# HansBambel/SmaAt-UNet

Measured on NVIDIA H100. Metric: SmaAt-UNet fwd frames/sec @ B=32 12×288×288; depthwise % HBM roofline, higher is better.
Workload: dtype f32

## Files before the change

### smaat_unet_b200/csrc/dsconv_fused.cu

```cuda
#include <stdlib.h>

#include "tc_common.cuh"

namespace smaat {

struct DsParams {
  const float* dw_w;
  const float* dw_b;
  const float* scale;
  const float* shift;
  float* y;
  int64_t y_bstride;
  double* stats;
  const float* oc_w;
  const float* oc_b;
  float* oc_y;
  int C0, C1, H, W, Cout, relu, K;
  int tiles_x, tiles_y, npass, total_tiles, nchunks;
};

template <int N_TILE, int KPL, int PW, bool X3>
struct DsCfg {
  static constexpr int PH = TC_BM / PW;
  static constexpr int BW = PW + 8, BH = PH + 2;
  static constexpr int CC = TC_BK / KPL;
  static constexpr int IN_BYTES = CC * BH * BW * 4;
  static constexpr int A_BYTES = TC_BM * TC_BK * 4;
  static constexpr int B_BYTES = N_TILE * TC_BK * 4;
  static constexpr int AST_BYTES = (X3 ? 2 : 1) * A_BYTES;
  static constexpr int BST_BYTES = (X3 ? 2 : 1) * B_BYTES;
  static constexpr int OFF_ALO = A_BYTES;
  static constexpr int OFF_BLO = B_BYTES;
  static constexpr int AS = X3 ? (N_TILE > 64 ? 2 : 3) : 4;
  static constexpr int NG = N_TILE > 64 ? 1 : 2;
  static constexpr int BS = X3 ? 2 : 4;
  static constexpr int AFF_N = 512;
  static constexpr int BAR_BYTES = 512;
  static constexpr int IS_FIT = (224 * 1024 - 1024 - BAR_BYTES - 3 * AFF_N * 4 - AS * AST_BYTES - BS * BST_BYTES) / IN_BYTES;
  static constexpr int IS = IS_FIT > 8 ? 8 : IS_FIT;
  static constexpr int OFF_A = ((IS * IN_BYTES + 1023) / 1024) * 1024;
  static constexpr int OFF_BR = OFF_A + AS * AST_BYTES;
  static constexpr int OFF_BAR = OFF_BR + BS * BST_BYTES;
  static_assert((IS * NG + IS + 2 * AS + 2 * BS) * 8 <= BAR_BYTES, "barrier block");
  static constexpr int TOTAL = OFF_BAR + BAR_BYTES + 3 * AFF_N * 4 + 1024;
  static constexpr uint32_t B_TX = BST_BYTES;
  static constexpr int PROD_WARP = 12;
  static constexpr int THREADS = 384 + 128 * NG;
  static_assert(IS >= 2, "input ring");
  static_assert(NG <= AS, "phase-parity barriers");
  static_assert(IN_BYTES % 128 == 0, "TMA destination alignment");
  static_assert(TOTAL <= 227 * 1024, "shared memory budget");
};

template <int N_TILE, int KPL, int PW, bool X3, bool A_SMEM>
__global__ void __launch_bounds__(DsCfg<N_TILE, KPL, PW, X3>::THREADS, 1)
    dsconv_fused_kernel(const __grid_constant__ CUtensorMap map_in0, const __grid_constant__ CUtensorMap map_in1,
                        const __grid_constant__ CUtensorMap map_w, const __grid_constant__ CUtensorMap map_wlo,
                        const DsParams p) {
  using L = DsCfg<N_TILE, KPL, PW, X3>;
  constexpr int PH = L::PH, BW = L::BW, BH = L::BH, CC = L::CC, IS = L::IS, AS = L::AS, BS = L::BS;
  extern __shared__ __align__(1024) unsigned char smem_dyn[];
  unsigned char* smem = smem_dyn + ((1024u - (smem_u32(smem_dyn) & 1023u)) & 1023u);
  unsigned char* a_base = smem + L::OFF_A;
  unsigned char* b_base = smem + L::OFF_BR;
  uint64_t* bars = reinterpret_cast<uint64_t*>(smem + L::OFF_BAR);
  uint64_t* in_full = bars;
  uint64_t* in_empty = in_full + IS * L::NG;
  uint64_t* a_full = in_empty + IS;
  uint64_t* a_empty = a_full + AS;
  uint64_t* b_full = a_empty + AS;
  uint64_t* b_empty = b_full + BS;
  float* aff = reinterpret_cast<float*>(smem + L::OFF_BAR + L::BAR_BYTES);

  const int warp = __shfl_sync(0xffffffffu, (int)(threadIdx.x >> 5), 0);
  const int lane = threadIdx.x & 31;
  const int nch = p.nchunks;
  const int tiles_per_img = p.tiles_x * p.tiles_y * p.npass;
  auto decode = [&](int tile, int& b, int& ty, int& tx, int& np) {
    b = tile / tiles_per_img;
    int t2 = tile - b * tiles_per_img;
    np = t2 % p.npass;
    t2 /= p.npass;
    ty = t2 / p.tiles_x;
    tx = t2 - ty * p.tiles_x;
  };

  if (warp == 0 && lane == 0) {
    tma_prefetch_desc(&map_in0);
    tma_prefetch_desc(&map_in1);
    tma_prefetch_desc(&map_w);
    if (X3) tma_prefetch_desc(&map_wlo);
    for (int s = 0; s < IS; ++s) {
      for (int g = 0; g < L::NG; ++g) mbar_init(&in_full[s * L::NG + g], 1);
      mbar_init(&in_empty[s], 128);
    }
    for (int s = 0; s < AS; ++s) {
      mbar_init(&a_full[s], 128);
      mbar_init(&a_empty[s], 8);
    }
    for (int s = 0; s < BS; ++s) {
      mbar_init(&b_full[s], 1);
      mbar_init(&b_empty[s], 8);
    }
    fence_barrier_init();
  }
  for (int c = threadIdx.x; c < L::AFF_N; c += blockDim.x) {
    aff[c] = (c < p.Cout && p.scale) ? __ldg(p.scale + c) : 1.f;
    aff[L::AFF_N + c] = (c < p.Cout && p.shift) ? __ldg(p.shift + c) : 0.f;
    aff[2 * L::AFF_N + c] = (c < p.Cout && p.oc_w) ? __ldg(p.oc_w + c) : 0.f;
  }
  __syncthreads();

  if (warp == 0) {
    if (lane == 0) {
      uint32_t gc = 0;
      for (int tile = blockIdx.x; tile < p.total_tiles; tile += gridDim.x) {
        int b, ty, tx, np;
        decode(tile, b, ty, tx, np);
        const int x0 = tx * PW, y0 = ty * PH;
        for (int i = 0; i < nch; ++i, ++gc) {
          const int s = gc % IS;
          mbar_wait(&in_empty[s], ((gc / IS) & 1u) ^ 1u);
          uint64_t* full = &in_full[s * L::NG + (int)(gc % (uint32_t)L::NG)];
          mbar_arrive_expect_tx(full, L::IN_BYTES);
          const int cb = i * CC;
          const CUtensorMap* m = (cb < p.C0) ? &map_in0 : &map_in1;
          const int cc = (cb < p.C0) ? cb : cb - p.C0;
          asm volatile(
              "cp.async.bulk.tensor.4d.shared::cluster.global.mbarrier::complete_tx::bytes [%0], [%1, {%3, %4, %5, %6}], [%2];" ::
                  "r"(smem_u32(smem + s * L::IN_BYTES)),
              "l"(reinterpret_cast<uint64_t>(m)), "r"(smem_u32(full)), "r"(x0 - 4), "r"(y0 - 1), "r"(cc), "r"(b)
              : "memory");
        }
      }
    }
    return;
  }
  if (warp == 1) {
    if (lane == 0) {
      uint32_t gc = 0;
      for (int tile = blockIdx.x; tile < p.total_tiles; tile += gridDim.x) {
        int b, ty, tx, np;
        decode(tile, b, ty, tx, np);
        for (int i = 0; i < nch; ++i, ++gc) {
          const int sb = gc % BS;
          mbar_wait(&b_empty[sb], ((gc / BS) & 1u) ^ 1u);
          mbar_arrive_expect_tx(&b_full[sb], L::B_TX);
          tma_load_2d(b_base + sb * L::BST_BYTES, &map_w, &b_full[sb], i * TC_BK, np * N_TILE);
          if (X3) tma_load_2d(b_base + sb * L::BST_BYTES + L::OFF_BLO, &map_wlo, &b_full[sb], i * TC_BK, np * N_TILE);
        }
      }
    }
    return;
  }
  if (warp < 4) return;

  if (warp < L::PROD_WARP) {
    const int wg = (warp >> 2) - 1, wq = warp & 3;
    const int g = lane >> 2, t = lane & 3;
    const int m0 = A_SMEM ? 64 * wg + 16 * wq + g : tc_row_pixel(wg, wq, 0, g);
    const int m1 = A_SMEM ? m0 + 8 : tc_row_pixel(wg, wq, 1, g);
    const float act_lo = p.relu ? 0.f : -INFINITY;
    const int64_t P = (int64_t)p.H * p.W;
    uint32_t gc = 0;
    for (int tile = blockIdx.x; tile < p.total_tiles; tile += gridDim.x) {
      int b, ty, tx, np;
      decode(tile, b, ty, tx, np);
      float acc[N_TILE / 2];
#pragma unroll
      for (int i = 0; i < N_TILE / 2; ++i) acc[i] = 0.f;
      for (int i = 0; i < nch; ++i, ++gc) {
        const int sa = gc % AS, sb = gc % BS;
        mbar_wait(&a_full[sa], (gc / AS) & 1u);
        mbar_wait(&b_full[sb], (gc / BS) & 1u);
        const unsigned char* ast = a_base + sa * L::AST_BYTES;
        const uint64_t bd0 = make_kmajor_desc(smem_u32(b_base + sb * L::BST_BYTES));
        const uint64_t bl0 = make_kmajor_desc(smem_u32(b_base + sb * L::BST_BYTES + L::OFF_BLO));
        if (A_SMEM) {
          const uint32_t a_addr = smem_u32(ast) + (uint32_t)(wg * 64 * 128);
          const uint64_t ad0 = make_kmajor_desc(a_addr), al0 = make_kmajor_desc(a_addr + L::OFF_ALO);
          wgmma_fence();
#pragma unroll
          for (int kk = 0; kk < TC_BK / 8; ++kk) {
            Wgmma<N_TILE>::ss(acc, ad0 + (uint64_t)(2 * kk), bd0 + (uint64_t)(2 * kk), 1u);
            if (X3) {
              Wgmma<N_TILE>::ss(acc, al0 + (uint64_t)(2 * kk), bd0 + (uint64_t)(2 * kk), 1u);
              Wgmma<N_TILE>::ss(acc, ad0 + (uint64_t)(2 * kk), bl0 + (uint64_t)(2 * kk), 1u);
            }
          }
        } else {
#pragma unroll
        for (int kk = 0; kk < TC_BK / 8; ++kk) {
          float vh[4], vl[4];
          load_a_frag(ast, kk, t, m0, m1, vh);
          if (X3) load_a_frag(ast + L::OFF_ALO, kk, t, m0, m1, vl);
          uint32_t ahi[4], alo[4];
#pragma unroll
          for (int e = 0; e < 4; ++e) {
            ahi[e] = __float_as_uint(vh[e]);
            alo[e] = X3 ? __float_as_uint(vl[e]) : 0u;
          }
          wgmma_fence();
          Wgmma<N_TILE>::rs(acc, ahi, bd0 + (uint64_t)(2 * kk), 1u);
          if (X3) {
            Wgmma<N_TILE>::rs(acc, alo, bd0 + (uint64_t)(2 * kk), 1u);
            Wgmma<N_TILE>::rs(acc, ahi, bl0 + (uint64_t)(2 * kk), 1u);
          }
        }
        }
        wgmma_commit();
        wgmma_wait0();
        wgmma_keep(acc);
        __syncwarp();
        if (lane == 0) {
          mbar_arrive(&a_empty[sa]);
          mbar_arrive(&b_empty[sb]);
        }
      }

      const int n0 = np * N_TILE;
      const int gy0 = ty * PH + m0 / PW, gx0 = tx * PW + m0 % PW;
      const int gy1 = ty * PH + m1 / PW, gx1 = tx * PW + m1 % PW;
      const bool v0 = gy0 < p.H && gx0 < p.W, v1 = gy1 < p.H && gx1 < p.W;
      const int64_t o0 = (int64_t)gy0 * p.W + gx0, o1 = (int64_t)gy1 * p.W + gx1;
      if (p.stats) {
        const double npix = (double)((__popc(__ballot_sync(0xffffffffu, v0)) + __popc(__ballot_sync(0xffffffffu, v1))) / 4);
#pragma unroll
        for (int j = 0; j < N_TILE / 8; ++j) {
#pragma unroll
          for (int e = 0; e < 2; ++e) {
            const float a = v0 ? acc[4 * j + e] : 0.f, bb = v1 ? acc[4 * j + 2 + e] : 0.f;
            const float s1 = frag_colsum(a + bb), s2 = frag_colsum(fmaf(a, a, bb * bb));
            const int c = 8 * j + 2 * t + e;
            if (lane < 4 && c < p.Cout) {
              const double sc = (double)aff[c], sh = (double)aff[L::AFF_N + c];
              atomicAdd(p.stats + c, sc * (double)s1 + npix * sh);
              atomicAdd(p.stats + p.Cout + c, sc * sc * (double)s2 + 2.0 * sc * sh * (double)s1 + npix * sh * sh);
            }
          }
        }
      }
      if (p.oc_y) {
        float d0 = 0.f, d1 = 0.f;
#pragma unroll
        for (int j = 0; j < N_TILE / 8; ++j) {
#pragma unroll
          for (int e = 0; e < 2; ++e) {
            const int c = 8 * j + 2 * t + e;
            const float sc = aff[c], sh = aff[L::AFF_N + c], w = aff[2 * L::AFF_N + c];
            d0 = fmaf(fmaxf(fmaf(acc[4 * j + e], sc, sh), act_lo), w, d0);
            d1 = fmaf(fmaxf(fmaf(acc[4 * j + 2 + e], sc, sh), act_lo), w, d1);
          }
        }
        d0 += __shfl_xor_sync(0xffffffffu, d0, 1);
        d0 += __shfl_xor_sync(0xffffffffu, d0, 2);
        d1 += __shfl_xor_sync(0xffffffffu, d1, 1);
        d1 += __shfl_xor_sync(0xffffffffu, d1, 2);
        const float ob = p.oc_b ? __ldg(p.oc_b) : 0.f;
        if (t == 0) {
          if (v0) p.oc_y[(int64_t)b * P + o0] = d0 + ob;
          if (v1) p.oc_y[(int64_t)b * P + o1] = d1 + ob;
        }
      } else {
        float* yb = p.y + (int64_t)b * p.y_bstride;
#pragma unroll
        for (int j = 0; j < N_TILE / 8; ++j) {
#pragma unroll
          for (int e = 0; e < 2; ++e) {
            const int c = n0 + 8 * j + 2 * t + e;
            if (c < p.Cout) {
              const float sc = aff[c], sh = aff[L::AFF_N + c];
              float* yc = yb + (int64_t)c * P;
              if (v0) yc[o0] = fmaxf(fmaf(acc[4 * j + e], sc, sh), act_lo);
              if (v1) yc[o1] = fmaxf(fmaf(acc[4 * j + 2 + e], sc, sh), act_lo);
            }
          }
        }
      }
    }
    return;
  }

  {
    const int g = (warp - L::PROD_WARP) >> 2;
    const int t = threadIdx.x - 32 * L::PROD_WARP - 128 * g;
    const int Cin = p.C0 + p.C1;
    uint32_t gc = 0, iph = 0;
    for (int tile = blockIdx.x; tile < p.total_tiles; tile += gridDim.x) {
      for (int i = 0; i < nch; ++i, ++gc) {
        if ((int)(gc % (uint32_t)L::NG) != g) continue;
        const int s = gc % IS;
        float wr[KPL][9], br[KPL];
        auto task_channel = [&](int task) { return (PW == 32) ? (task >> 3) : (((task >> 4) << 1) | ((task >> 2) & 1)); };
        auto load_weights = [&](int task) {
          const int gch = i * CC + task_channel(task);
          const bool chv = gch < Cin;
#pragma unroll
          for (int kk = 0; kk < KPL; ++kk) {
            const int gk = gch * KPL + kk;
#pragma unroll
            for (int w9 = 0; w9 < 9; ++w9) wr[kk][w9] = chv ? __ldg(p.dw_w + (int64_t)gk * 9 + w9) : 0.f;
            br[kk] = (chv && p.dw_b) ? __ldg(p.dw_b + gk) : 0.f;
          }
        };
        load_weights(t);
        mbar_wait(&in_full[s * L::NG + g], (iph >> s) & 1u);
        iph ^= 1u << s;
        const int sa = gc % AS;
        mbar_wait(&a_empty[sa], ((gc / AS) & 1u) ^ 1u);
        unsigned char* my_op = a_base + sa * L::AST_BYTES;
        const float* in_stage = reinterpret_cast<const float*>(smem + s * L::IN_BYTES);
#pragma unroll 1
        for (int task = t; task < CC * 8; task += 128) {
          int ci, qc, rg;
          if (PW == 32) {
            ci = task >> 3; qc = task & 7; rg = 0;
          } else {
            qc = task & 3; ci = ((task >> 4) << 1) | ((task >> 2) & 1); rg = (task >> 3) & 1;
          }
          constexpr int NQ = PW / 4;
          const int c0 = qc << 2, r0 = rg << 2;
          if (task != t) load_weights(task);
          const float* trow = in_stage + (ci * BH + r0) * BW + c0 + 3;
          float win[3][6];
          const bool lb = (qc == 0), rb = (qc == NQ - 1);
          const int edge = lb ? 0 : 5;
          auto load_row = [&](float* wl, int r) {
            const float4 a = *reinterpret_cast<const float4*>(trow + r * BW + 1);
            float left = __shfl_up_sync(0xffffffffu, a.w, 1), right = __shfl_down_sync(0xffffffffu, a.x, 1);
            if (lb | rb) {
              const float e = trow[r * BW + edge];
              if (lb) left = e; else right = e;
            }
            wl[0] = left; wl[1] = a.x; wl[2] = a.y; wl[3] = a.z; wl[4] = a.w; wl[5] = right;
          };
#pragma unroll
          for (int r = 0; r < 2; ++r) load_row(win[r], r);
#pragma unroll
          for (int rr = 0; rr < 4; ++rr) {
            load_row(win[(rr + 2) % 3], rr + 2);
            const float* w0 = win[rr % 3];
            const float* w1 = win[(rr + 1) % 3];
            const float* w2 = win[(rr + 2) % 3];
            const int m = (r0 + rr) * PW + c0;
#pragma unroll
            for (int kk = 0; kk < KPL; ++kk) {
              float o4[4];
#pragma unroll
              for (int j = 0; j < 4; ++j) {
                float a = br[kk];
                a = fmaf(wr[kk][0], w0[j], a); a = fmaf(wr[kk][1], w0[j + 1], a); a = fmaf(wr[kk][2], w0[j + 2], a);
                a = fmaf(wr[kk][3], w1[j], a); a = fmaf(wr[kk][4], w1[j + 1], a); a = fmaf(wr[kk][5], w1[j + 2], a);
                a = fmaf(wr[kk][6], w2[j], a); a = fmaf(wr[kk][7], w2[j + 1], a); a = fmaf(wr[kk][8], w2[j + 2], a);
                o4[j] = a;
              }
              if (A_SMEM) {
                const int kr = ci * KPL + kk;
#pragma unroll
                for (int j = 0; j < 4; ++j) {
                  const uint32_t off = kmajor_offset(m + j, kr);
                  const float h = X3 ? tf32_hi(o4[j]) : o4[j];
                  *reinterpret_cast<float*>(my_op + off) = h;
                  if (X3) *reinterpret_cast<float*>(my_op + L::OFF_ALO + off) = o4[j] - h;
                }
                continue;
              }
              const uint32_t off = a_tile_offset(ci * KPL + kk, m);
              if (X3) {
                const float4 h = make_float4(tf32_hi(o4[0]), tf32_hi(o4[1]), tf32_hi(o4[2]), tf32_hi(o4[3]));
                *reinterpret_cast<float4*>(my_op + off) = h;
                *reinterpret_cast<float4*>(my_op + L::OFF_ALO + off) = make_float4(o4[0] - h.x, o4[1] - h.y, o4[2] - h.z, o4[3] - h.w);
              } else {
                *reinterpret_cast<float4*>(my_op + off) = make_float4(o4[0], o4[1], o4[2], o4[3]);
              }
            }
          }
        }
        if (A_SMEM) fence_proxy_async_smem();
        mbar_arrive(&a_full[sa]);
        mbar_arrive(&in_empty[s]);
      }
    }
  }
}

template <int N_TILE, int KPL, int PW, bool X3, bool A_SMEM>
static int launch_ds(const CUtensorMap& m0, const CUtensorMap& m1, const CUtensorMap& mw, const CUtensorMap& mwl, DsParams p,
                     int B, cudaStream_t st) {
  using L = DsCfg<N_TILE, KPL, PW, X3>;
  auto kern = dsconv_fused_kernel<N_TILE, KPL, PW, X3, A_SMEM>;
  static std::atomic<uint64_t> attr_mask{0};
  if (first_use_on_device(attr_mask)) {
    cudaError_t e = cudaFuncSetAttribute(kern, cudaFuncAttributeMaxDynamicSharedMemorySize, L::TOTAL);
    if (e != cudaSuccess) return fail(SMAAT_E_CUDA, "dsconv: smem attribute (%d B): %s", L::TOTAL, cudaGetErrorString(e));
  }
  p.tiles_x = ceil_div(p.W, PW);
  p.tiles_y = ceil_div(p.H, L::PH);
  p.npass = ceil_div(p.Cout, N_TILE);
  const int64_t total = (int64_t)B * p.tiles_x * p.tiles_y * p.npass;
  SMAAT_REQUIRE(total < (1ll << 31), "dsconv: too many tiles");
  p.total_tiles = (int)total;
  p.nchunks = ceil_div(p.C0 + p.C1, L::CC);
  const int grid = p.total_tiles < num_sms() ? p.total_tiles : num_sms();
  kern<<<grid, L::THREADS, L::TOTAL, st>>>(m0, m1, mw, mwl, p);
  SMAAT_LAUNCH_CHECK("smaat_dsconv_fwd");
  return SMAAT_OK;
}

static int pick_pw(int H, int W) {
  double best = 1e9;
  int pw = 0;
  const int cand[2] = {32, 16};
  for (int i = 0; i < 2; ++i) {
    const int c = cand[i], ph = TC_BM / c;
    const double waste = ((double)ceil_div(W, c) * c / W) * ((double)ceil_div(H, ph) * ph / H);
    if (waste < best - 1e-9) {
      best = waste;
      pw = c;
    }
  }
  return best <= 1.35 ? pw : 0;
}

static bool ds_eligible(const float* x0, int C0, int64_t bs0, const float* x1, int C1, int64_t bs1, const float* pw_w,
                        const float* pw_w_lo, int H, int W, int k, int Cout, bool stats, bool outconv) {
  if (k != 1 && k != 2) return false;
  if (Cout < 8 || Cout > 512 || (Cout > 128 && (Cout % 128 != 0 || stats || outconv))) return false;
  if (W % 4 != 0 || !aligned16(x0) || bs0 % 4 != 0) return false;
  if (C1 > 0 && (!aligned16(x1) || bs1 % 4 != 0 || C0 % (TC_BK / k) != 0)) return false;
  const int K = k * (C0 + C1);
  if (K % 4 != 0 || !aligned16(pw_w) || (pw_w_lo && !aligned16(pw_w_lo))) return false;
  return pick_pw(H, W) != 0;
}

static std::atomic<int> g_ds_impl{-1};
static int ds_impl() {
  int v = g_ds_impl.load(std::memory_order_relaxed);
  if (v < 0) {
    const char* e = getenv("SMAAT_DS_IMPL");
    v = e ? atoi(e) : 0;
    if (v < 0 || v > 2) v = 0;
    g_ds_impl.store(v, std::memory_order_relaxed);
  }
  return v;
}

}

using namespace smaat;

extern "C" int smaat_set_dsconv_impl(int impl) {
  SMAAT_REQUIRE(impl >= 0 && impl <= 2, "set_dsconv_impl: 0 = auto, 1 = A operand from shared memory, 2 = A operand from registers");
  g_ds_impl.store(impl, std::memory_order_relaxed);
  return SMAAT_OK;
}

extern "C" int smaat_dsconv_eligible2(const float* x0, int C0, int64_t x0_bstride, const float* x1, int C1, int64_t x1_bstride,
                                      const float* pw_w, int H, int W, int k, int Cout, int with_stats) {
  return ds_eligible(x0, C0, x0_bstride, x1, C1, x1_bstride, pw_w, nullptr, H, W, k, Cout, with_stats != 0, false) ? 1 : 0;
}

extern "C" int smaat_dsconv_eligible(const float* x0, int C0, int64_t x0_bstride, const float* x1, int C1, int64_t x1_bstride,
                                     const float* pw_w, int H, int W, int k, int Cout) {
  return smaat_dsconv_eligible2(x0, C0, x0_bstride, x1, C1, x1_bstride, pw_w, H, W, k, Cout, 0);
}

static int dsconv_run(const float* x0, int C0, int64_t x0_bstride, const float* x1, int C1, int64_t x1_bstride, const float* dw_w,
                      const float* dw_b, const float* pw_w, const float* pw_w_lo, const float* scale, const float* shift, float* y,
                      int64_t y_bstride, double* stats, const float* oc_w, const float* oc_b, float* oc_y, int B, int H, int W,
                      int k, int Cout, int relu, int mode, void* stream) {
  SMAAT_REQUIRE(x0 && dw_w && pw_w && (y || oc_y), "dsconv: null pointer");
  SMAAT_REQUIRE(B > 0 && C0 > 0 && C1 >= 0 && H > 0 && W > 0 && Cout > 0, "dsconv: bad shape");
  SMAAT_REQUIRE(C1 == 0 || x1, "dsconv: C1=%d but x1 is null", C1);
  SMAAT_REQUIRE(mode == SMAAT_PW_TF32 || mode == SMAAT_PW_TF32X3, "dsconv: mode must be SMAAT_PW_TF32 or SMAAT_PW_TF32X3");
  SMAAT_REQUIRE(mode != SMAAT_PW_TF32X3 || pw_w_lo, "dsconv: TF32X3 needs pw_w_lo (see smaat_split_tf32)");
  SMAAT_REQUIRE(oc_y || y_bstride >= (int64_t)Cout * H * W, "dsconv: y batch stride too small");
  SMAAT_REQUIRE(!oc_y || (oc_w && !stats), "dsconv+outconv: needs the OutConv weight and no batch statistics");
  if (!ds_eligible(x0, C0, x0_bstride, x1, C1, x1_bstride, pw_w, pw_w_lo, H, W, k, Cout, stats != nullptr, oc_y != nullptr))
    return fail(SMAAT_E_UNSUPPORTED, "dsconv: shape not taken by the fused kernel (k=%d Cout=%d H=%d W=%d); use dw3x3 + pw1x1", k,
                Cout, H, W);
  cudaStream_t st = (cudaStream_t)stream;
  const int pw = pick_pw(H, W);
  const int ph = TC_BM / pw;
  const int n_tile = Cout > 64 ? 128 : 64;
  const int cc = TC_BK / k;
  const bool x3 = mode == SMAAT_PW_TF32X3;
  const bool a_smem = ds_impl() == 1;
  const int K = k * (C0 + C1);

  CUtensorMap m0, m1, mw, mwl;
  const uint32_t box[4] = {(uint32_t)(pw + 8), (uint32_t)(ph + 2), (uint32_t)cc, 1u};
  {
    const uint64_t dims[4] = {(uint64_t)W, (uint64_t)H, (uint64_t)C0, (uint64_t)B};
    const uint64_t str[4] = {0, (uint64_t)W * 4, (uint64_t)H * W * 4, (uint64_t)x0_bstride * 4};
    int r = make_tmap_f32(&m0, x0, 4, dims, str, box, CU_TENSOR_MAP_SWIZZLE_NONE, "dsconv(x0)");
    if (r) return r;
    m1 = m0;
  }
  if (C1 > 0) {
    const uint64_t dims[4] = {(uint64_t)W, (uint64_t)H, (uint64_t)C1, (uint64_t)B};
    const uint64_t str[4] = {0, (uint64_t)W * 4, (uint64_t)H * W * 4, (uint64_t)x1_bstride * 4};
    int r = make_tmap_f32(&m1, x1, 4, dims, str, box, CU_TENSOR_MAP_SWIZZLE_NONE, "dsconv(x1)");
    if (r) return r;
  }
  {
    const uint64_t dims[2] = {(uint64_t)K, (uint64_t)Cout};
    const uint64_t str[2] = {0, (uint64_t)K * 4};
    const uint32_t wbox[2] = {(uint32_t)TC_BK, (uint32_t)n_tile};
    int r = make_tmap_f32(&mw, pw_w, 2, dims, str, wbox, CU_TENSOR_MAP_SWIZZLE_128B, "dsconv(w)");
    if (r) return r;
    mwl = mw;
    if (x3) {
      r = make_tmap_f32(&mwl, pw_w_lo, 2, dims, str, wbox, CU_TENSOR_MAP_SWIZZLE_128B, "dsconv(w_lo)");
      if (r) return r;
    }
  }
  DsParams p;
  p.dw_w = dw_w; p.dw_b = dw_b; p.scale = scale; p.shift = shift; p.y = y; p.y_bstride = y_bstride; p.stats = stats;
  p.oc_w = oc_w; p.oc_b = oc_b; p.oc_y = oc_y;
  p.C0 = C0; p.C1 = C1; p.H = H; p.W = W; p.Cout = Cout; p.relu = relu; p.K = K;
  p.tiles_x = p.tiles_y = p.npass = p.total_tiles = p.nchunks = 0;

#define DS_DISPATCH(NT, KP, PWv)                                                                           \
  return x3 ? (a_smem ? launch_ds<NT, KP, PWv, true, true>(m0, m1, mw, mwl, p, B, st)                       \
                      : launch_ds<NT, KP, PWv, true, false>(m0, m1, mw, mwl, p, B, st))                     \
            : (a_smem ? launch_ds<NT, KP, PWv, false, true>(m0, m1, mw, mwl, p, B, st)                      \
                      : launch_ds<NT, KP, PWv, false, false>(m0, m1, mw, mwl, p, B, st))
  if (n_tile == 64) {
    if (k == 2) { if (pw == 32) { DS_DISPATCH(64, 2, 32); } else { DS_DISPATCH(64, 2, 16); } }
    else        { if (pw == 32) { DS_DISPATCH(64, 1, 32); } else { DS_DISPATCH(64, 1, 16); } }
  } else {
    if (k == 2) { if (pw == 32) { DS_DISPATCH(128, 2, 32); } else { DS_DISPATCH(128, 2, 16); } }
    else        { if (pw == 32) { DS_DISPATCH(128, 1, 32); } else { DS_DISPATCH(128, 1, 16); } }
  }
#undef DS_DISPATCH
}

extern "C" int smaat_dsconv_fwd(const float* x0, int C0, int64_t x0_bstride, const float* x1, int C1, int64_t x1_bstride,
                                const float* dw_w, const float* dw_b, const float* pw_w, const float* pw_w_lo,
                                const float* scale, const float* shift, float* y, int64_t y_bstride, double* stats, int B, int H,
                                int W, int k, int Cout, int relu, int mode, void* stream) {
  SMAAT_REQUIRE(y, "dsconv: null output");
  return dsconv_run(x0, C0, x0_bstride, x1, C1, x1_bstride, dw_w, dw_b, pw_w, pw_w_lo, scale, shift, y, y_bstride, stats, nullptr,
                    nullptr, nullptr, B, H, W, k, Cout, relu, mode, stream);
}

extern "C" int smaat_dsconv_outconv_fwd(const float* x0, int C0, int64_t x0_bstride, const float* x1, int C1, int64_t x1_bstride,
                                        const float* dw_w, const float* dw_b, const float* pw_w, const float* pw_w_lo,
                                        const float* scale, const float* shift, const float* oc_w, const float* oc_b,
                                        float* logits, int B, int H, int W, int k, int Cout, int relu, int mode, void* stream) {
  SMAAT_REQUIRE(oc_w && logits, "dsconv+outconv: null pointer");
  return dsconv_run(x0, C0, x0_bstride, x1, C1, x1_bstride, dw_w, dw_b, pw_w, pw_w_lo, scale, shift, nullptr, 0, nullptr, oc_w, oc_b,
                    logits, B, H, W, k, Cout, relu, mode, stream);
}
```

### smaat_unet_b200/csrc/pw1x1_tc.cu

```cuda
#include <stdlib.h>

#include "tc_common.cuh"

namespace smaat {

struct PwTcParams {
  const float* scale;
  const float* shift;
  float* y;
  int64_t y_bstride;
  double* stats;
  int K, Cout, P, relu;
  int tiles_m, tiles_n, total_tiles;
};

template <int N_TILE, int STAGES, bool X3>
struct PwTcCfg {
  static constexpr int A_BYTES = TC_BM * TC_BK * 4;
  static constexpr int B_BYTES = N_TILE * TC_BK * 4;
  static constexpr int STAGE_BYTES = A_BYTES + (X3 ? 2 : 1) * B_BYTES;
  static constexpr int OFF_B = A_BYTES;
  static constexpr int OFF_BLO = A_BYTES + B_BYTES;
  static constexpr int BAR_BYTES = 256;
  static constexpr int AFF_N = 512;
  static constexpr int SACC_BYTES = 8 * 2 * N_TILE * 8;
  static constexpr int TOTAL = STAGES * STAGE_BYTES + BAR_BYTES + 2 * AFF_N * 4 + SACC_BYTES + 1024;
  static constexpr uint32_t TX_BYTES = A_BYTES + (X3 ? 2 : 1) * B_BYTES;
  static constexpr int THREADS = 384;
  static_assert(TOTAL <= 227 * 1024, "shared memory budget");
};

template <int N_TILE, int STAGES, bool X3>
__global__ void __launch_bounds__(384, 1)
    pw1x1_tc_kernel(const __grid_constant__ CUtensorMap map_x, const __grid_constant__ CUtensorMap map_w,
                    const __grid_constant__ CUtensorMap map_wlo, const PwTcParams p) {
  using L = PwTcCfg<N_TILE, STAGES, X3>;
  extern __shared__ __align__(1024) unsigned char smem_dyn[];
  unsigned char* smem = smem_dyn + ((1024u - (smem_u32(smem_dyn) & 1023u)) & 1023u);
  uint64_t* bars = reinterpret_cast<uint64_t*>(smem + STAGES * L::STAGE_BYTES);
  float* aff = reinterpret_cast<float*>(smem + STAGES * L::STAGE_BYTES + L::BAR_BYTES);
  uint64_t* full_bar = bars;
  uint64_t* empty_bar = bars + STAGES;

  const int warp = __shfl_sync(0xffffffffu, (int)(threadIdx.x >> 5), 0);
  const int lane = threadIdx.x & 31;
  const int nk = (p.K + TC_BK - 1) / TC_BK;

  if (warp == 0 && lane == 0) {
    tma_prefetch_desc(&map_x);
    tma_prefetch_desc(&map_w);
    if (X3) tma_prefetch_desc(&map_wlo);
    for (int s = 0; s < STAGES; ++s) {
      mbar_init(&full_bar[s], 1);
      mbar_init(&empty_bar[s], 8);
    }
    fence_barrier_init();
  }
  for (int c = threadIdx.x; c < L::AFF_N; c += blockDim.x) {
    aff[c] = (c < p.Cout && p.scale) ? __ldg(p.scale + c) : 1.f;
    aff[L::AFF_N + c] = (c < p.Cout && p.shift) ? __ldg(p.shift + c) : 0.f;
  }
  __syncthreads();

  if (warp == 0) {
    if (lane == 0) {
      uint32_t it = 0;
      for (int tile = blockIdx.x; tile < p.total_tiles; tile += gridDim.x) {
        const int tn = tile % p.tiles_n;
        const int rest = tile / p.tiles_n;
        const int tm = rest % p.tiles_m;
        const int b = rest / p.tiles_m;
        const int p0 = tm * TC_BM, n0 = tn * N_TILE;
        for (int i = 0; i < nk; ++i, ++it) {
          const int s = it % STAGES;
          const uint32_t ph = (it / STAGES) & 1u;
          mbar_wait(&empty_bar[s], ph ^ 1u);
          unsigned char* st = smem + s * L::STAGE_BYTES;
          mbar_arrive_expect_tx(&full_bar[s], L::TX_BYTES);
          const int k0 = i * TC_BK;
#pragma unroll
          for (int j = 0; j < 4; ++j) tma_load_3d(st + j * (TC_BK * 128), &map_x, &full_bar[s], p0 + 32 * j, k0, b);
          tma_load_2d(st + L::OFF_B, &map_w, &full_bar[s], k0, n0);
          if (X3) tma_load_2d(st + L::OFF_BLO, &map_wlo, &full_bar[s], k0, n0);
        }
      }
    }
    return;
  }
  if (warp < 4) return;

  const int wg = (warp >> 2) - 1, wq = warp & 3, cw = warp - 4;
  const int g = lane >> 2, t = lane & 3;
  const int m0 = tc_row_pixel(wg, wq, 0, g), m1 = tc_row_pixel(wg, wq, 1, g);
  const float act_lo = p.relu ? 0.f : -INFINITY;
  double* sacc = reinterpret_cast<double*>(smem + STAGES * L::STAGE_BYTES + L::BAR_BYTES + 2 * L::AFF_N * 4) + cw * 2 * N_TILE;
  int stat_n0 = -1;
  if (p.stats) {
    for (int c = lane; c < 2 * N_TILE; c += 32) sacc[c] = 0.0;
    __syncwarp();
  }
  double stat_npix = 0.0;
  auto flush_stats = [&](int n0f) {
    __syncwarp();
    for (int c = lane; c < N_TILE; c += 32) {
      if (n0f + c < p.Cout) {
        const double sc = (double)aff[(n0f + c) & (L::AFF_N - 1)], sh = (double)aff[L::AFF_N + ((n0f + c) & (L::AFF_N - 1))];
        const double S1 = sacc[c], S2 = sacc[N_TILE + c];
        atomicAdd(p.stats + n0f + c, sc * S1 + stat_npix * sh);
        atomicAdd(p.stats + p.Cout + n0f + c, sc * sc * S2 + 2.0 * sc * sh * S1 + stat_npix * sh * sh);
      }
      sacc[c] = 0.0;
      sacc[N_TILE + c] = 0.0;
    }
    stat_npix = 0.0;
    __syncwarp();
  };

  uint32_t it = 0;
  for (int tile = blockIdx.x; tile < p.total_tiles; tile += gridDim.x) {
    const int tn = tile % p.tiles_n;
    const int rest = tile / p.tiles_n;
    const int tm = rest % p.tiles_m;
    const int b = rest / p.tiles_m;
    const int n0 = tn * N_TILE;
    if (p.stats && n0 != stat_n0) {
      if (stat_n0 >= 0) flush_stats(stat_n0);
      stat_n0 = n0;
    }
    float acc[N_TILE / 2];
#pragma unroll
    for (int i = 0; i < N_TILE / 2; ++i) acc[i] = 0.f;
    for (int i = 0; i < nk; ++i, ++it) {
      const int s = it % STAGES;
      mbar_wait(&full_bar[s], (it / STAGES) & 1u);
      const unsigned char* st = smem + s * L::STAGE_BYTES;
      const uint64_t bd0 = make_kmajor_desc(smem_u32(st + L::OFF_B));
      const uint64_t bl0 = make_kmajor_desc(smem_u32(st + L::OFF_BLO));
#pragma unroll
      for (int kk = 0; kk < TC_BK / 8; ++kk) {
        float v[4];
        load_a_frag(st, kk, t, m0, m1, v);
        uint32_t ahi[4], alo[4];
#pragma unroll
        for (int e = 0; e < 4; ++e) {
          const float h = X3 ? tf32_hi(v[e]) : v[e];
          ahi[e] = __float_as_uint(h);
          alo[e] = __float_as_uint(v[e] - h);
        }
        wgmma_fence();
        Wgmma<N_TILE>::rs(acc, ahi, bd0 + (uint64_t)(2 * kk), 1u);
        if (X3) {
          Wgmma<N_TILE>::rs(acc, alo, bd0 + (uint64_t)(2 * kk), 1u);
          Wgmma<N_TILE>::rs(acc, ahi, bl0 + (uint64_t)(2 * kk), 1u);
        }
      }
      wgmma_commit();
      wgmma_wait0();
      wgmma_keep(acc);
      __syncwarp();
      if (lane == 0) mbar_arrive(&empty_bar[s]);
    }

    const int pix0 = tm * TC_BM + m0, pix1 = tm * TC_BM + m1;
    const bool v0 = pix0 < p.P, v1 = pix1 < p.P;
    float* yb = p.y + (int64_t)b * p.y_bstride;
#pragma unroll
    for (int j = 0; j < N_TILE / 8; ++j) {
#pragma unroll
      for (int e = 0; e < 2; ++e) {
        const int c = n0 + 8 * j + 2 * t + e;
        if (c < p.Cout) {
          const float sc = aff[c & (L::AFF_N - 1)], sh = aff[L::AFF_N + (c & (L::AFF_N - 1))];
          float* yc = yb + (int64_t)c * p.P;
          if (v0) yc[pix0] = fmaxf(fmaf(acc[4 * j + e], sc, sh), act_lo);
          if (v1) yc[pix1] = fmaxf(fmaf(acc[4 * j + 2 + e], sc, sh), act_lo);
        }
      }
    }
    if (p.stats) {
#pragma unroll
      for (int j = 0; j < N_TILE / 8; ++j) {
#pragma unroll
        for (int e = 0; e < 2; ++e) {
          const float a = acc[4 * j + e], bb = acc[4 * j + 2 + e];
          const float s1 = frag_colsum(a + bb), s2 = frag_colsum(fmaf(a, a, bb * bb));
          if (lane < 4) {
            const int col = 8 * j + 2 * t + e;
            sacc[col] += (double)s1;
            sacc[N_TILE + col] += (double)s2;
          }
        }
      }
      const int nv = __popc(__ballot_sync(0xffffffffu, v0)) + __popc(__ballot_sync(0xffffffffu, v1));
      stat_npix += (double)(nv / 4);
    }
  }
  if (p.stats && stat_n0 >= 0) flush_stats(stat_n0);
}

template <int N_TILE, int STAGES, bool X3>
static int launch_tc(const CUtensorMap& mx, const CUtensorMap& mw, const CUtensorMap& mwl, PwTcParams p, int B, cudaStream_t st) {
  using L = PwTcCfg<N_TILE, STAGES, X3>;
  auto kern = pw1x1_tc_kernel<N_TILE, STAGES, X3>;
  static std::atomic<uint64_t> attr_mask{0};
  if (first_use_on_device(attr_mask)) {
    cudaError_t e = cudaFuncSetAttribute(kern, cudaFuncAttributeMaxDynamicSharedMemorySize, L::TOTAL);
    if (e != cudaSuccess) return fail(SMAAT_E_CUDA, "pw1x1(tc): smem attribute (%d B): %s", L::TOTAL, cudaGetErrorString(e));
  }
  p.tiles_m = ceil_div(p.P, TC_BM);
  p.tiles_n = ceil_div(p.Cout, N_TILE);
  const int64_t total = (int64_t)B * p.tiles_m * p.tiles_n;
  SMAAT_REQUIRE(total < (1ll << 31), "pw1x1(tc): too many tiles");
  p.total_tiles = (int)total;
  const int grid = p.total_tiles < num_sms() ? p.total_tiles : num_sms();
  kern<<<grid, L::THREADS, L::TOTAL, st>>>(mx, mw, mwl, p);
  SMAAT_LAUNCH_CHECK("smaat_pw1x1_fwd(tc)");
  return SMAAT_OK;
}

bool pw1x1_tc_eligible(const float* x, const float* w, const float* w_lo, int K, int Cout, int P) {
  return (P % 4 == 0) && (K % 4 == 0) && aligned16(x) && aligned16(w) && (w_lo == nullptr || aligned16(w_lo)) && Cout >= 8;
}

int pw1x1_tc_launch(const float* x, const float* w, const float* w_lo, const float* scale, const float* shift, float* y,
                    int64_t y_bstride, double* stats, int B, int K, int Cout, int P, int relu, bool x3, cudaStream_t st) {
  SMAAT_REQUIRE(pw1x1_tc_eligible(x, w, w_lo, K, Cout, P), "pw1x1(tc): needs P %% 4 == 0, K %% 4 == 0 and 16-byte aligned x/w");
  SMAAT_REQUIRE(!x3 || w_lo, "pw1x1(tc): TF32X3 needs w_lo (see smaat_split_tf32)");
  SMAAT_REQUIRE(Cout <= 512 || (!scale && !shift), "pw1x1(tc): Cout=%d > 512 with an epilogue affine (smem staging holds 512 channels)", Cout);
  const int n_tile = Cout > 64 ? 128 : 64;

  CUtensorMap mx, mw, mwl;
  {
    const uint64_t dims[3] = {(uint64_t)P, (uint64_t)K, (uint64_t)B};
    const uint64_t str[3] = {0, (uint64_t)P * 4, (uint64_t)K * P * 4};
    const uint32_t box[3] = {32u, (uint32_t)TC_BK, 1u};
    int r = make_tmap_f32(&mx, x, 3, dims, str, box, CU_TENSOR_MAP_SWIZZLE_128B, "pw1x1(x)");
    if (r) return r;
  }
  {
    const uint64_t dims[2] = {(uint64_t)K, (uint64_t)Cout};
    const uint64_t str[2] = {0, (uint64_t)K * 4};
    const uint32_t box[2] = {(uint32_t)TC_BK, (uint32_t)n_tile};
    int r = make_tmap_f32(&mw, w, 2, dims, str, box, CU_TENSOR_MAP_SWIZZLE_128B, "pw1x1(w)");
    if (r) return r;
    mwl = mw;
    if (x3) {
      r = make_tmap_f32(&mwl, w_lo, 2, dims, str, box, CU_TENSOR_MAP_SWIZZLE_128B, "pw1x1(w_lo)");
      if (r) return r;
    }
  }
  PwTcParams p;
  p.scale = scale; p.shift = shift; p.y = y; p.y_bstride = y_bstride; p.stats = stats;
  p.K = K; p.Cout = Cout; p.P = P; p.relu = relu;
  p.tiles_m = p.tiles_n = p.total_tiles = 0;

  if (x3) {
    if (n_tile == 128) return launch_tc<128, 3, true>(mx, mw, mwl, p, B, st);
    return launch_tc<64, 5, true>(mx, mw, mwl, p, B, st);
  }
  if (n_tile == 128) return launch_tc<128, 5, false>(mx, mw, mwl, p, B, st);
  return launch_tc<64, 6, false>(mx, mw, mwl, p, B, st);
}

}
```

### smaat_unet_b200/csrc/tc_common.cuh

```cuda
#pragma once
#include "common.cuh"
#include "wgmma.cuh"

namespace smaat {

constexpr int TC_BM = 128;
constexpr int TC_BK = 32;

__device__ __forceinline__ void wgmma_fence() { asm volatile("wgmma.fence.sync.aligned;" ::: "memory"); }
__device__ __forceinline__ void wgmma_commit() { asm volatile("wgmma.commit_group.sync.aligned;" ::: "memory"); }
__device__ __forceinline__ void wgmma_wait0() { asm volatile("wgmma.wait_group.sync.aligned 0;" ::: "memory"); }
template <int N>
__device__ __forceinline__ void wgmma_keep(float (&d)[N]) {
#pragma unroll
  for (int i = 0; i < N; ++i) asm volatile("" : "+f"(d[i])::"memory");
}

__device__ __forceinline__ uint64_t make_kmajor_desc(uint32_t saddr) {
  uint64_t d = 0;
  d |= (uint64_t)((saddr >> 4) & 0x3fffu);
  d |= (uint64_t)1 << 16;
  d |= (uint64_t)(1024 >> 4) << 32;
  d |= (uint64_t)1 << 62;
  return d;
}

__device__ __forceinline__ uint32_t a_tile_offset(int kr, int m) {
  const int j = m >> 5, col = m & 31;
  return (uint32_t)(j * (TC_BK * 128) + kr * 128 + ((((col >> 2) ^ (kr & 7)) << 4) | ((col & 3) << 2)));
}

__device__ __forceinline__ uint32_t kmajor_offset(int row, int k) {
  return (uint32_t)(row * 128 + ((((k >> 2) ^ (row & 7)) << 4) | ((k & 3) << 2)));
}

__device__ __forceinline__ int tc_row_pixel(int wg, int wq, int e, int g) {
  return 64 * wg + 32 * (wq >> 1) + 4 * (2 * (wq & 1) + e) + (g & 3) + 16 * (g >> 2);
}

__device__ __forceinline__ void load_a_frag(const unsigned char* at, int kk, int t, int m0, int m1, float (&v)[4]) {
  const int k0 = 8 * kk + t;
  v[0] = *reinterpret_cast<const float*>(at + a_tile_offset(k0, m0));
  v[1] = *reinterpret_cast<const float*>(at + a_tile_offset(k0, m1));
  v[2] = *reinterpret_cast<const float*>(at + a_tile_offset(k0 + 4, m0));
  v[3] = *reinterpret_cast<const float*>(at + a_tile_offset(k0 + 4, m1));
}

__device__ __forceinline__ float tf32_hi(float v) { return __uint_as_float(__float_as_uint(v) & 0xffffe000u); }

__device__ __forceinline__ float frag_colsum(float v) {
  v += __shfl_xor_sync(0xffffffffu, v, 4);
  v += __shfl_xor_sync(0xffffffffu, v, 8);
  v += __shfl_xor_sync(0xffffffffu, v, 16);
  return v;
}

__device__ __forceinline__ void consumer_sync() { asm volatile("bar.sync 1, 256;" ::: "memory"); }

}
```

Measured before the change: 2380.

## Overlap wgmma groups with fragment loads and rebalance warpgroup registers via setmaxnreg

The wgmma consumers in the fused depthwise-separable and 1x1 tensor-core kernels now keep one committed wgmma group in flight (wait_group 1). The next chunk's A fragments are loaded into a ping-pong register buffer and stage buffers are released one iteration late, instead of fully draining after every K chunk. Registers are moved from the TMA warps (and the producer warpgroup when N_TILE>64) to the MMA warps with setmaxnreg. The X3 hi/lo TF32 split of the register-fed A operand moves from the depthwise producer into the consumer. Stage counts are also retuned, and a host-side check rejects builds whose register count cannot cover the split. In exchange the consumers carry more register pressure, and the deferred release logic adds complexity in how buffers are returned.

```diff
diff --git a/smaat_unet_b200/csrc/dsconv_fused.cu b/smaat_unet_b200/csrc/dsconv_fused.cu
--- a/smaat_unet_b200/csrc/dsconv_fused.cu
+++ b/smaat_unet_b200/csrc/dsconv_fused.cu
@@ -19,7 +19,7 @@
   int tiles_x, tiles_y, npass, total_tiles, nchunks;
 };
 
-template <int N_TILE, int KPL, int PW, bool X3>
+template <int N_TILE, int KPL, int PW, bool X3, bool A_SMEM>
 struct DsCfg {
   static constexpr int PH = TC_BM / PW;
   static constexpr int BW = PW + 8, BH = PH + 2;
@@ -27,13 +27,13 @@
   static constexpr int IN_BYTES = CC * BH * BW * 4;
   static constexpr int A_BYTES = TC_BM * TC_BK * 4;
   static constexpr int B_BYTES = N_TILE * TC_BK * 4;
-  static constexpr int AST_BYTES = (X3 ? 2 : 1) * A_BYTES;
+  static constexpr int AST_BYTES = (X3 && A_SMEM ? 2 : 1) * A_BYTES;
   static constexpr int BST_BYTES = (X3 ? 2 : 1) * B_BYTES;
   static constexpr int OFF_ALO = A_BYTES;
   static constexpr int OFF_BLO = B_BYTES;
-  static constexpr int AS = X3 ? (N_TILE > 64 ? 2 : 3) : 4;
   static constexpr int NG = N_TILE > 64 ? 1 : 2;
-  static constexpr int BS = X3 ? 2 : 4;
+  static constexpr int AS = X3 ? (A_SMEM ? (N_TILE > 64 ? 2 : 3) : 2 + NG) : 4;
+  static constexpr int BS = X3 ? (A_SMEM && N_TILE > 64 ? 2 : 3) : 4;
   static constexpr int AFF_N = 512;
   static constexpr int BAR_BYTES = 512;
   static constexpr int IS_FIT = (224 * 1024 - 1024 - BAR_BYTES - 3 * AFF_N * 4 - AS * AST_BYTES - BS * BST_BYTES) / IN_BYTES;
@@ -46,6 +46,13 @@
   static constexpr uint32_t B_TX = BST_BYTES;
   static constexpr int PROD_WARP = 12;
   static constexpr int THREADS = 384 + 128 * NG;
+  static constexpr int REGS_LAUNCH = (65536 / THREADS) / 8 * 8;
+  static constexpr int REGS_TMA = 24;
+  static constexpr int REGS_PROD = N_TILE > 64 ? 104 : REGS_LAUNCH;
+  static constexpr int REGS_MMA = ((THREADS / 128 * REGS_LAUNCH - REGS_TMA - NG * REGS_PROD) / 2) / 8 * 8;
+  static constexpr int REGS_SUM = REGS_TMA + 2 * REGS_MMA + NG * REGS_PROD;
+  static_assert(REGS_SUM <= THREADS / 128 * REGS_LAUNCH && REGS_MMA >= REGS_LAUNCH, "register budget");
+  static constexpr int KS = (X3 && N_TILE == 64) ? 2 : TC_BK / 8;
   static_assert(IS >= 2, "input ring");
   static_assert(NG <= AS, "phase-parity barriers");
   static_assert(IN_BYTES % 128 == 0, "TMA destination alignment");
@@ -53,11 +60,11 @@
 };
 
 template <int N_TILE, int KPL, int PW, bool X3, bool A_SMEM>
-__global__ void __launch_bounds__(DsCfg<N_TILE, KPL, PW, X3>::THREADS, 1)
+__global__ void __launch_bounds__(DsCfg<N_TILE, KPL, PW, X3, A_SMEM>::THREADS, 1)
     dsconv_fused_kernel(const __grid_constant__ CUtensorMap map_in0, const __grid_constant__ CUtensorMap map_in1,
                         const __grid_constant__ CUtensorMap map_w, const __grid_constant__ CUtensorMap map_wlo,
                         const DsParams p) {
-  using L = DsCfg<N_TILE, KPL, PW, X3>;
+  using L = DsCfg<N_TILE, KPL, PW, X3, A_SMEM>;
   constexpr int PH = L::PH, BW = L::BW, BH = L::BH, CC = L::CC, IS = L::IS, AS = L::AS, BS = L::BS;
   extern __shared__ __align__(1024) unsigned char smem_dyn[];
   unsigned char* smem = smem_dyn + ((1024u - (smem_u32(smem_dyn) & 1023u)) & 1023u);
@@ -111,8 +118,9 @@
   }
   __syncthreads();
 
-  if (warp == 0) {
-    if (lane == 0) {
+  if (warp < 4) {
+    regs_dealloc<L::REGS_TMA>();
+    if (warp == 0 && lane == 0) {
       uint32_t gc = 0;
       for (int tile = blockIdx.x; tile < p.total_tiles; tile += gridDim.x) {
         int b, ty, tx, np;
@@ -134,10 +142,7 @@
         }
       }
     }
-    return;
-  }
-  if (warp == 1) {
-    if (lane == 0) {
+    if (warp == 1 && lane == 0) {
       uint32_t gc = 0;
       for (int tile = blockIdx.x; tile < p.total_tiles; tile += gridDim.x) {
         int b, ty, tx, np;
@@ -153,9 +158,9 @@
     }
     return;
   }
-  if (warp < 4) return;
 
   if (warp < L::PROD_WARP) {
+    regs_alloc<L::REGS_MMA>();
     const int wg = (warp >> 2) - 1, wq = warp & 3;
     const int g = lane >> 2, t = lane & 3;
     const int m0 = A_SMEM ? 64 * wg + 16 * wq + g : tc_row_pixel(wg, wq, 0, g);
@@ -169,14 +174,26 @@
       float acc[N_TILE / 2];
 #pragma unroll
       for (int i = 0; i < N_TILE / 2; ++i) acc[i] = 0.f;
-      for (int i = 0; i < nch; ++i, ++gc) {
+      auto release = [&](uint32_t c) {
+        __syncwarp();
+        if (lane == 0) {
+          mbar_arrive(&a_empty[c % AS]);
+          mbar_arrive(&b_empty[c % BS]);
+        }
+      };
+      auto wait_stages = [&](const unsigned char*& ast, uint64_t& bd, uint64_t& bl) {
         const int sa = gc % AS, sb = gc % BS;
         mbar_wait(&a_full[sa], (gc / AS) & 1u);
         mbar_wait(&b_full[sb], (gc / BS) & 1u);
-        const unsigned char* ast = a_base + sa * L::AST_BYTES;
-        const uint64_t bd0 = make_kmajor_desc(smem_u32(b_base + sb * L::BST_BYTES));
-        const uint64_t bl0 = make_kmajor_desc(smem_u32(b_base + sb * L::BST_BYTES + L::OFF_BLO));
-        if (A_SMEM) {
+        ast = a_base + sa * L::AST_BYTES;
+        bd = make_kmajor_desc(smem_u32(b_base + sb * L::BST_BYTES));
+        bl = make_kmajor_desc(smem_u32(b_base + sb * L::BST_BYTES + L::OFF_BLO));
+      };
+      if (A_SMEM) {
+        for (int i = 0; i < nch; ++i, ++gc) {
+          const unsigned char* ast;
+          uint64_t bd0, bl0;
+          wait_stages(ast, bd0, bl0);
           const uint32_t a_addr = smem_u32(ast) + (uint32_t)(wg * 64 * 128);
           const uint64_t ad0 = make_kmajor_desc(a_addr), al0 = make_kmajor_desc(a_addr + L::OFF_ALO);
           wgmma_fence();
@@ -188,35 +205,39 @@
               Wgmma<N_TILE>::ss(acc, ad0 + (uint64_t)(2 * kk), bl0 + (uint64_t)(2 * kk), 1u);
             }
           }
-        } else {
-#pragma unroll
-        for (int kk = 0; kk < TC_BK / 8; ++kk) {
-          float vh[4], vl[4];
-          load_a_frag(ast, kk, t, m0, m1, vh);
-          if (X3) load_a_frag(ast + L::OFF_ALO, kk, t, m0, m1, vl);
-          uint32_t ahi[4], alo[4];
-#pragma unroll
-          for (int e = 0; e < 4; ++e) {
-            ahi[e] = __float_as_uint(vh[e]);
-            alo[e] = X3 ? __float_as_uint(vl[e]) : 0u;
-          }
-          wgmma_fence();
-          Wgmma<N_TILE>::rs(acc, ahi, bd0 + (uint64_t)(2 * kk), 1u);
-          if (X3) {
-            Wgmma<N_TILE>::rs(acc, alo, bd0 + (uint64_t)(2 * kk), 1u);
-            Wgmma<N_TILE>::rs(acc, ahi, bl0 + (uint64_t)(2 * kk), 1u);
-          }
-        }
-        }
-        wgmma_commit();
+          wgmma_commit();
+          wgmma_wait<1>();
+          if (i > 0) release(gc - 1);
+        }
         wgmma_wait0();
-        wgmma_keep(acc);
-        __syncwarp();
-        if (lane == 0) {
-          mbar_arrive(&a_empty[sa]);
-          mbar_arrive(&b_empty[sb]);
-        }
+      } else {
+        constexpr int KS = L::KS, GPC = (TC_BK / 8) / KS;
+        const unsigned char* ast = nullptr;
+        uint64_t bd0 = 0, bl0 = 0;
+        auto group = [&](AFrags<X3, KS>& cur, AFrags<X3, KS>& prev, int q) {
+          const int part = q % GPC;
+          if (part == 0) wait_stages(ast, bd0, bl0);
+          load_a_frags<X3, KS>(ast, part * KS, t, m0, m1, cur);
+          mma_a_frags<N_TILE, X3, KS>(acc, cur, bd0, bl0, part * KS);
+          wgmma_wait<1>();
+          wgmma_keep(prev);
+          if (part == 0 && q > 0) release(gc - 1);
+          if (part == GPC - 1) ++gc;
+        };
+        AFrags<X3, KS> fa, fb;
+        const int ngrp = nch * GPC;
+        int q = 0;
+        for (; q + 1 < ngrp; q += 2) {
+          group(fa, fb, q);
+          group(fb, fa, q + 1);
+        }
+        if (q < ngrp) group(fa, fb, q);
+        wgmma_wait0();
+        wgmma_keep(fa);
+        wgmma_keep(fb);
       }
+      wgmma_keep(acc);
+      release(gc - 1);
 
       const int n0 = np * N_TILE;
       const int gy0 = ty * PH + m0 / PW, gx0 = tx * PW + m0 % PW;
@@ -282,6 +303,7 @@
   }
 
   {
+    if (L::REGS_PROD < L::REGS_LAUNCH) regs_dealloc<L::REGS_PROD>();
     const int g = (warp - L::PROD_WARP) >> 2;
     const int t = threadIdx.x - 32 * L::PROD_WARP - 128 * g;
     const int Cin = p.C0 + p.C1;
@@ -365,14 +387,7 @@
                 }
                 continue;
               }
-              const uint32_t off = a_tile_offset(ci * KPL + kk, m);
-              if (X3) {
-                const float4 h = make_float4(tf32_hi(o4[0]), tf32_hi(o4[1]), tf32_hi(o4[2]), tf32_hi(o4[3]));
-                *reinterpret_cast<float4*>(my_op + off) = h;
-                *reinterpret_cast<float4*>(my_op + L::OFF_ALO + off) = make_float4(o4[0] - h.x, o4[1] - h.y, o4[2] - h.z, o4[3] - h.w);
-              } else {
-                *reinterpret_cast<float4*>(my_op + off) = make_float4(o4[0], o4[1], o4[2], o4[3]);
-              }
+              *reinterpret_cast<float4*>(my_op + a_tile_offset(ci * KPL + kk, m)) = make_float4(o4[0], o4[1], o4[2], o4[3]);
             }
           }
         }
@@ -387,12 +402,14 @@
 template <int N_TILE, int KPL, int PW, bool X3, bool A_SMEM>
 static int launch_ds(const CUtensorMap& m0, const CUtensorMap& m1, const CUtensorMap& mw, const CUtensorMap& mwl, DsParams p,
                      int B, cudaStream_t st) {
-  using L = DsCfg<N_TILE, KPL, PW, X3>;
+  using L = DsCfg<N_TILE, KPL, PW, X3, A_SMEM>;
   auto kern = dsconv_fused_kernel<N_TILE, KPL, PW, X3, A_SMEM>;
   static std::atomic<uint64_t> attr_mask{0};
   if (first_use_on_device(attr_mask)) {
     cudaError_t e = cudaFuncSetAttribute(kern, cudaFuncAttributeMaxDynamicSharedMemorySize, L::TOTAL);
     if (e != cudaSuccess) return fail(SMAAT_E_CUDA, "dsconv: smem attribute (%d B): %s", L::TOTAL, cudaGetErrorString(e));
+    int r = check_reg_budget((const void*)kern, L::THREADS, L::REGS_SUM, "dsconv");
+    if (r) return r;
   }
   p.tiles_x = ceil_div(p.W, PW);
   p.tiles_y = ceil_div(p.H, L::PH);
diff --git a/smaat_unet_b200/csrc/pw1x1_tc.cu b/smaat_unet_b200/csrc/pw1x1_tc.cu
--- a/smaat_unet_b200/csrc/pw1x1_tc.cu
+++ b/smaat_unet_b200/csrc/pw1x1_tc.cu
@@ -27,6 +27,9 @@
   static constexpr int TOTAL = STAGES * STAGE_BYTES + BAR_BYTES + 2 * AFF_N * 4 + SACC_BYTES + 1024;
   static constexpr uint32_t TX_BYTES = A_BYTES + (X3 ? 2 : 1) * B_BYTES;
   static constexpr int THREADS = 384;
+  static constexpr int REGS_TMA = 40, REGS_MMA = 232;
+  static_assert(REGS_TMA + 2 * REGS_MMA <= 3 * 168, "register budget");
+  static_assert(STAGES >= 3, "ring depth");
   static_assert(TOTAL <= 227 * 1024, "shared memory budget");
 };
 
@@ -62,8 +65,9 @@
   }
   __syncthreads();
 
-  if (warp == 0) {
-    if (lane == 0) {
+  if (warp < 4) {
+    regs_dealloc<L::REGS_TMA>();
+    if (warp == 0 && lane == 0) {
       uint32_t it = 0;
       for (int tile = blockIdx.x; tile < p.total_tiles; tile += gridDim.x) {
         const int tn = tile % p.tiles_n;
@@ -87,7 +91,7 @@
     }
     return;
   }
-  if (warp < 4) return;
+  regs_alloc<L::REGS_MMA>();
 
   const int wg = (warp >> 2) - 1, wq = warp & 3, cw = warp - 4;
   const int g = lane >> 2, t = lane & 3;
@@ -130,36 +134,34 @@
     float acc[N_TILE / 2];
 #pragma unroll
     for (int i = 0; i < N_TILE / 2; ++i) acc[i] = 0.f;
-    for (int i = 0; i < nk; ++i, ++it) {
+    auto release = [&](uint32_t c) {
+      __syncwarp();
+      if (lane == 0) mbar_arrive(&empty_bar[c % STAGES]);
+    };
+    auto chunk = [&](AFrags<X3>& cur, AFrags<X3>& prev, int i) {
       const int s = it % STAGES;
       mbar_wait(&full_bar[s], (it / STAGES) & 1u);
       const unsigned char* st = smem + s * L::STAGE_BYTES;
-      const uint64_t bd0 = make_kmajor_desc(smem_u32(st + L::OFF_B));
-      const uint64_t bl0 = make_kmajor_desc(smem_u32(st + L::OFF_BLO));
-#pragma unroll
-      for (int kk = 0; kk < TC_BK / 8; ++kk) {
-        float v[4];
-        load_a_frag(st, kk, t, m0, m1, v);
-        uint32_t ahi[4], alo[4];
-#pragma unroll
-        for (int e = 0; e < 4; ++e) {
-          const float h = X3 ? tf32_hi(v[e]) : v[e];
-          ahi[e] = __float_as_uint(h);
-          alo[e] = __float_as_uint(v[e] - h);
-        }
-        wgmma_fence();
-        Wgmma<N_TILE>::rs(acc, ahi, bd0 + (uint64_t)(2 * kk), 1u);
-        if (X3) {
-          Wgmma<N_TILE>::rs(acc, alo, bd0 + (uint64_t)(2 * kk), 1u);
-          Wgmma<N_TILE>::rs(acc, ahi, bl0 + (uint64_t)(2 * kk), 1u);
-        }
-      }
-      wgmma_commit();
-      wgmma_wait0();
-      wgmma_keep(acc);
-      __syncwarp();
-      if (lane == 0) mbar_arrive(&empty_bar[s]);
-    }
+      load_a_frags<X3, TC_BK / 8>(st, 0, t, m0, m1, cur);
+      mma_a_frags<N_TILE, X3, TC_BK / 8>(acc, cur, make_kmajor_desc(smem_u32(st + L::OFF_B)),
+                                         make_kmajor_desc(smem_u32(st + L::OFF_BLO)), 0);
+      wgmma_wait<1>();
+      wgmma_keep(prev);
+      if (i > 0) release(it - 1);
+      ++it;
+    };
+    AFrags<X3> fa, fb;
+    int i = 0;
+    for (; i + 1 < nk; i += 2) {
+      chunk(fa, fb, i);
+      chunk(fb, fa, i + 1);
+    }
+    if (i < nk) chunk(fa, fb, i);
+    wgmma_wait0();
+    wgmma_keep(acc);
+    wgmma_keep(fa);
+    wgmma_keep(fb);
+    release(it - 1);
 
     const int pix0 = tm * TC_BM + m0, pix1 = tm * TC_BM + m1;
     const bool v0 = pix0 < p.P, v1 = pix1 < p.P;
@@ -206,6 +208,8 @@
   if (first_use_on_device(attr_mask)) {
     cudaError_t e = cudaFuncSetAttribute(kern, cudaFuncAttributeMaxDynamicSharedMemorySize, L::TOTAL);
     if (e != cudaSuccess) return fail(SMAAT_E_CUDA, "pw1x1(tc): smem attribute (%d B): %s", L::TOTAL, cudaGetErrorString(e));
+    int r = check_reg_budget((const void*)kern, L::THREADS, L::REGS_TMA + 2 * L::REGS_MMA, "pw1x1(tc)");
+    if (r) return r;
   }
   p.tiles_m = ceil_div(p.P, TC_BM);
   p.tiles_n = ceil_div(p.Cout, N_TILE);
@@ -255,7 +259,7 @@
   p.tiles_m = p.tiles_n = p.total_tiles = 0;
 
   if (x3) {
-    if (n_tile == 128) return launch_tc<128, 3, true>(mx, mw, mwl, p, B, st);
+    if (n_tile == 128) return launch_tc<128, 4, true>(mx, mw, mwl, p, B, st);
     return launch_tc<64, 5, true>(mx, mw, mwl, p, B, st);
   }
   if (n_tile == 128) return launch_tc<128, 5, false>(mx, mw, mwl, p, B, st);
diff --git a/smaat_unet_b200/csrc/tc_common.cuh b/smaat_unet_b200/csrc/tc_common.cuh
--- a/smaat_unet_b200/csrc/tc_common.cuh
+++ b/smaat_unet_b200/csrc/tc_common.cuh
@@ -11,9 +11,36 @@
 __device__ __forceinline__ void wgmma_commit() { asm volatile("wgmma.commit_group.sync.aligned;" ::: "memory"); }
 __device__ __forceinline__ void wgmma_wait0() { asm volatile("wgmma.wait_group.sync.aligned 0;" ::: "memory"); }
 template <int N>
+__device__ __forceinline__ void wgmma_wait() { asm volatile("wgmma.wait_group.sync.aligned %0;" ::"n"(N) : "memory"); }
+template <int N>
 __device__ __forceinline__ void wgmma_keep(float (&d)[N]) {
 #pragma unroll
   for (int i = 0; i < N; ++i) asm volatile("" : "+f"(d[i])::"memory");
+}
+template <int P, int K>
+__device__ __forceinline__ void wgmma_keep(uint32_t (&a)[P][K][4]) {
+#pragma unroll
+  for (int p = 0; p < P; ++p)
+#pragma unroll
+    for (int k = 0; k < K; ++k)
+#pragma unroll
+      for (int e = 0; e < 4; ++e) asm volatile("" : "+r"(a[p][k][e])::"memory");
+}
+
+template <int R>
+__device__ __forceinline__ void regs_dealloc() { asm volatile("setmaxnreg.dec.sync.aligned.u32 %0;" ::"n"(R)); }
+template <int R>
+__device__ __forceinline__ void regs_alloc() { asm volatile("setmaxnreg.inc.sync.aligned.u32 %0;" ::"n"(R)); }
+
+inline int check_reg_budget(const void* kern, int threads, int regs_sum, const char* who) {
+  cudaFuncAttributes a;
+  cudaError_t e = cudaFuncGetAttributes(&a, kern);
+  if (e != cudaSuccess) return fail(SMAAT_E_CUDA, "%s: cudaFuncGetAttributes: %s", who, cudaGetErrorString(e));
+  const int launched = ((a.numRegs + 7) / 8) * 8 * (threads / 128);
+  if (launched < regs_sum)
+    return fail(SMAAT_E_CUDA, "%s: built with %d registers per thread, the warpgroups' register split needs %d per 128 threads > %d",
+                who, a.numRegs, regs_sum, launched);
+  return SMAAT_OK;
 }
 
 __device__ __forceinline__ uint64_t make_kmajor_desc(uint32_t saddr) {
@@ -48,6 +75,39 @@
 
 __device__ __forceinline__ float tf32_hi(float v) { return __uint_as_float(__float_as_uint(v) & 0xffffe000u); }
 
+template <bool X3, int KS = TC_BK / 8>
+using AFrags = uint32_t[X3 ? 2 : 1][KS][4];
+
+template <bool X3, int KS>
+__device__ __forceinline__ void load_a_frags(const unsigned char* at, int kk0, int t, int m0, int m1, AFrags<X3, KS>& f) {
+#pragma unroll
+  for (int kk = 0; kk < KS; ++kk) {
+    float v[4];
+    load_a_frag(at, kk0 + kk, t, m0, m1, v);
+#pragma unroll
+    for (int e = 0; e < 4; ++e) {
+      const float h = X3 ? tf32_hi(v[e]) : v[e];
+      f[0][kk][e] = __float_as_uint(h);
+      if (X3) f[X3 ? 1 : 0][kk][e] = __float_as_uint(v[e] - h);
+    }
+  }
+}
+
+template <int N_TILE, bool X3, int KS>
+__device__ __forceinline__ void mma_a_frags(float (&acc)[N_TILE / 2], const AFrags<X3, KS>& f, uint64_t bd, uint64_t bl, int kk0) {
+  wgmma_fence();
+#pragma unroll
+  for (int kk = 0; kk < KS; ++kk) {
+    const uint64_t k2 = (uint64_t)(2 * (kk0 + kk));
+    Wgmma<N_TILE>::rs(acc, f[0][kk], bd + k2, 1u);
+    if (X3) {
+      Wgmma<N_TILE>::rs(acc, f[X3 ? 1 : 0][kk], bd + k2, 1u);
+      Wgmma<N_TILE>::rs(acc, f[0][kk], bl + k2, 1u);
+    }
+  }
+  wgmma_commit();
+}
+
 __device__ __forceinline__ float frag_colsum(float v) {
   v += __shfl_xor_sync(0xffffffffu, v, 4);
   v += __shfl_xor_sync(0xffffffffu, v, 8);
```

New measurement: 2486, median of 6. 1.04x the previous value.
